# BoChenUIUC/FastVideoCodec

Measured on AMD Instinct MI355X. Metric: 1080p frames/sec encode+decode at λ=1024; bpp/PSNR parity vs CPU ref, higher is better.
Workload: dtype f32 (convs: fp32 operands split into fp16 hi/lo, f32 accumulate); 1 GPU; DVC P-frame encode+decode with rANS, 1920x1080 (padded 1920x1088) GOP-12, lambda=1024 slot; gops_per_gpu=16, frames_counted=P-frames only (I-frame pass-through), parallelism=gop-shard x1

## Files before the change

### fastvideocodec_amd/csrc/fvc_conv_x3.hip

```cpp
#include "fvc_common.h"
#include "fvc_dx.h"
#include <math.h>
#include <stdlib.h>

namespace {

#ifndef FVC_STORE_AUX
#define FVC_STORE_AUX 0
#endif

typedef _Float16 h8 __attribute__((ext_vector_type(8)));

constexpr int kMaxTapsX = 49;

constexpr float kLoScale = 2048.f;
#ifndef FVC_X3_KO
#define FVC_X3_KO 0
#endif
constexpr int kKO = FVC_X3_KO;
#ifndef FVC_X3_SCHED
#define FVC_X3_SCHED 0
#endif
constexpr int kSched = FVC_X3_SCHED;
#ifndef FVC_X3_ACC1
// ... 688 lines not shown
        for (int ky = 0; ky < ks; ++ky) {
          if (((py + pad - ky) % stride + stride) % stride) continue;
          for (int kx = 0; kx < ks; ++kx) {
            if (((px + pad - kx) % stride + stride) % stride) continue;
            const int t = c.ntaps[cl]++;
            c.tky[cl][t] = ky; c.tkx[cl][t] = kx;
            c.tdy[cl][t] = x3_floordiv(py + pad - ky, stride);
            c.tdx[cl][t] = x3_floordiv(px + pad - kx, stride);
          }
        }
      }
  }
  c.dymin = c.dxmin = 1 << 20;
  c.dymax = c.dxmax = -(1 << 20);
  for (int cl = 0; cl < c.nclass; ++cl)
    for (int t = 0; t < c.ntaps[cl]; ++t) {
      c.dymin = c.tdy[cl][t] < c.dymin ? c.tdy[cl][t] : c.dymin;
      c.dymax = c.tdy[cl][t] > c.dymax ? c.tdy[cl][t] : c.dymax;
      c.dxmin = c.tdx[cl][t] < c.dxmin ? c.tdx[cl][t] : c.dxmin;
      c.dxmax = c.tdx[cl][t] > c.dxmax ? c.tdx[cl][t] : c.dxmax;
    }
  c.dx = 0;
  c.wl = 0;
  if (transposed && stride == 2 && c.nclass == 4 && env_int("FVC_DX", 1) &&
      (c.cinp == 64 || c.cinp == 96 || c.cinp == 128) && (c.ntp == 2 || c.ntp == 4)) {
    int maxt = 0;
    for (int cl = 0; cl < 4; ++cl) maxt = c.ntaps[cl] > maxt ? c.ntaps[cl] : maxt;
    const int sw = fvc_dx::strip_width(c.cinp);
    const int R = sw == 16 ? 8 : (c.ntp == 4 ? 2 : 4);
    const int ir = R + (c.dymax - c.dymin), ic = sw + (c.dxmax - c.dxmin);
    if (maxt <= fvc_dx::kMaxTaps && fvc_dx::lds_bytes(c.cinp, fvc_dx::plane_pix(ir, ic)) <= 160 * 1024) {
      c.dx = 1;
      c.cc = c.cinp;
      c.nchunks = 1;
      c.nw = 8;
      c.wm = 2;
      c.wn = 2;
      c.wnmax = 2;
      c.th = R;
      long long off = 0;
      for (int cl = 0; cl < 4; ++cl) {
        c.nks[cl] = fvc_cdiv(c.ntaps[cl] * (c.cc / 8), 2);
        c.wcls[cl] = off;
        off += (long long)c.nks[cl] * c.ntp * kFrag;
      }
      c.wtotal = off;
      return true;
    }
  }
  c.cc = (c.cinp % 32 == 0) ? 32 : ((c.cinp % 16 == 0) ? 16 : 8);
  const int want_cc = env_int("FVC_X3_CC", 0);
  if ((want_cc == 8 || want_cc == 16 || want_cc == 32) && c.cinp % want_cc == 0) c.cc = want_cc;
  c.nw = 8;
  c.wm = env_int("FVC_X3_WM", (!transposed && stride == 2) ? 1 : 2) == 1 ? 1 : 2;
  c.wl = env_int("FVC_X3_WL", 0) ? 1 : 0;
  c.wnmax = (c.wm == 1 && !transposed && stride == 2 && c.ntp % 4 == 0) ? 4 : (c.ntp >= 2 ? 2 : 1);
  for (;;) {
    c.th = c.nw * c.wm;
    const int ir = (c.th - 1) * c.sin + 1 + (c.dymax - c.dymin);
    const int ic = 31 * c.sin + 1 + (c.dxmax - c.dxmin);
    size_t lds = 1024 + 2 * x3_tile_bytes(ir, ic, c.cc);
    if (c.wl) {
      int nkmax = 0;
      for (int cl = 0; cl < c.nclass; ++cl) {
        const int nk = fvc_cdiv(c.ntaps[cl] * (c.cc / 8), 2);
        nkmax = nk > nkmax ? nk : nkmax;
      }
      lds += 2 * (size_t)nkmax * c.wnmax * kFrag * 16;
    }
    if (lds <= 160 * 1024) break;
    if (c.cc > 8 && c.cinp % (c.cc / 2) == 0) c.cc /= 2;
    else if (c.wm > 1) c.wm /= 2;
    else return false;
  }
  c.nchunks = c.cinp == 4 ? 1 : c.cinp / c.cc;
  c.wn = 1;
  long long off = 0;
  for (int cl = 0; cl < c.nclass; ++cl) {
    c.nks[cl] = fvc_cdiv(c.ntaps[cl] * (c.cc / 8), 2);
    c.wcls[cl] = off;
    off += (long long)c.nchunks * c.nks[cl] * c.ntp * kFrag;
  }
  c.wtotal = off;
  return true;
}

static int x3_num_cus() {
  static int n = 0;
  if (!n) {
    int dev = 0;
    if (hipGetDevice(&dev) != hipSuccess ||
        hipDeviceGetAttribute(&n, hipDeviceAttributeMultiprocessorCount, dev) != hipSuccess || n <= 0)
      n = 256;
  }
  return n;
}

static int x3_kw(const float* w, size_t n) {
  float mx = 0.f;
  for (size_t i = 0; i < n; ++i) mx = fabsf(w[i]) > mx ? fabsf(w[i]) : mx;
  if (!(mx > 0.f) || !isfinite(mx)) return 0;
  int e;
  frexpf(mx, &e);
  int kw = 14 - e;
  return kw < -100 ? -100 : (kw > 100 ? 100 : kw);
}

template <int CC, int WM, int WN, int WG, int IOP, int POST, int NWV, int WL>
static int x3_launch(const X3Args& a, dim3 grid, size_t lds, hipStream_t s) {
  if (lds > 64 * 1024)
    (void)hipFuncSetAttribute((const void*)conv_x3_kernel<CC, WM, WN, WG, IOP, POST, NWV, WL>,
                              hipFuncAttributeMaxDynamicSharedMemorySize, (int)lds);
  hipLaunchKernelGGL((conv_x3_kernel<CC, WM, WN, WG, IOP, POST, NWV, WL>), grid, dim3(NWV * 64), lds, s, a);
  FVC_CHECK_LAUNCH();
  return 0;
}

template <int CC, int WM, int WN, int WG, int WL, int NWV = 8>
static int x3_launch_iop(int iop, int post, const X3Args& a, dim3 grid, size_t lds, hipStream_t s) {
  if (post == kPostPool) {
    if constexpr (WG == 1 && WL == 0 && WM == 2 && WN <= 2)
      return iop == FVC_IN_NONE ? x3_launch<CC, WM, WN, WG, FVC_IN_NONE, kPostPool, NWV, WL>(a, grid, lds, s) : FVC_EINVAL;
    return FVC_EINVAL;
  }
  if (post == kPostTap) {
    if constexpr (WG == 1 && WL == 0 && ((WM == 2 && WN <= 2) || (WM == 1 && WN == 4)))
      return iop == FVC_IN_NONE ? x3_launch<CC, WM, WN, WG, FVC_IN_NONE, kPostTap, NWV, WL>(a, grid, lds, s) : FVC_EINVAL;
    return FVC_EINVAL;
  }
  if (post == FVC_POST_EXP)
    return iop == FVC_IN_NONE ? x3_launch<CC, WM, WN, WG, FVC_IN_NONE, FVC_POST_EXP, NWV, WL>(a, grid, lds, s) : FVC_EINVAL;
  switch (iop) {
    case FVC_IN_NONE: return x3_launch<CC, WM, WN, WG, FVC_IN_NONE, FVC_POST_NONE, NWV, WL>(a, grid, lds, s);
    case FVC_IN_RELU: return x3_launch<CC, WM, WN, WG, FVC_IN_RELU, FVC_POST_NONE, NWV, WL>(a, grid, lds, s);
    case FVC_IN_ABS: return x3_launch<CC, WM, WN, WG, FVC_IN_ABS, FVC_POST_NONE, NWV, WL>(a, grid, lds, s);
    case FVC_IN_ROUND: return x3_launch<CC, WM, WN, WG, FVC_IN_ROUND, FVC_POST_NONE, NWV, WL>(a, grid, lds, s);
  }
  return FVC_EINVAL;
}

template <int CC, int WL>
static int x3_launch_cc(int nwv, int wm, int wn, int wg, int iop, int post, const X3Args& a, dim3 grid,
                        size_t lds, hipStream_t s) {
  if (nwv != 8) return FVC_EINVAL;
  if (wg == 2) return (wm == 4 && wn == 1 && !WL) ? x3_launch_iop<CC, 4, 1, 2, 0>(iop, post, a, grid, lds, s) : FVC_EINVAL;
  if (wm == 2 && wn == 2) return x3_launch_iop<CC, 2, 2, 1, WL>(iop, post, a, grid, lds, s);
  if (wm == 2 && wn == 1) return x3_launch_iop<CC, 2, 1, 1, WL>(iop, post, a, grid, lds, s);
  if (wm == 1 && wn == 2) return x3_launch_iop<CC, 1, 2, 1, WL>(iop, post, a, grid, lds, s);
  if (wm == 1 && wn == 1) return x3_launch_iop<CC, 1, 1, 1, WL>(iop, post, a, grid, lds, s);
  if (wm == 1 && wn == 4) return x3_launch_iop<CC, 1, 4, 1, WL>(iop, post, a, grid, lds, s);
  return FVC_EINVAL;
}

static int run_dx(const X3Cfg& c, const float* x, const void* wpack, float osc, const float* bias, const float* res,
                  float* y, int batch, int h, int w, int cout, int in_op, int act, int post_op, int cu_reserve,
                  int* ovf, int* sched, int sched_len, hipStream_t s, const void* tw, float tosc, int pcp,
                  unsigned y_bytes, unsigned x_bytes) {
  const bool tap = tw != nullptr;
  if (tap && res) return FVC_EINVAL;
  const int R = c.th;
  const int sw = fvc_dx::strip_width(c.cinp);
  const int S = R / (32 / sw);
  const int wm = tap ? 1 : 2, wn = tap ? c.ntp : 2;
  fvc_dx::DxArgs d;
  d.x = x;
  d.w = (const uint4*)wpack;
  d.bias = bias;
  d.res = res;
  d.y = y;
  d.post_exp = post_op == FVC_POST_EXP ? 1 : 0;
  d.B = batch;
  d.H = h;
  d.W = w;
  d.cout = cout;
  d.coutp = c.coutp;
  d.ntp = c.ntp;
  d.R = R;
  d.sw = sw;
  d.ir = R + (c.dymax - c.dymin);
  d.ic = sw + (c.dxmax - c.dxmin);
  d.ps = fvc_dx::plane_pix(d.ir, d.ic);
  d.dymin = c.dymin;
  d.dxmin = c.dxmin;
  d.inv_ic = 1.0f / (float)d.ic;
  d.tiles_x = fvc_cdiv(w, sw);
  d.tiles_y = fvc_cdiv(h, R);
  const long long nitems = (long long)batch * d.tiles_x * d.tiles_y;
  if (nitems >= (1LL << 30)) return FVC_EINVAL;
  d.nitems = (int)nitems;
  d.osc = osc;
  d.osc_c = osc * (1.0f / 2048.f);
  d.act_slope = act == FVC_ACT_RELU ? 0.f : (act == FVC_ACT_LRELU ? 0.1f : 1.f);
  for (int cl = 0; cl < 4; ++cl) {
    d.nks[cl] = c.nks[cl];
    d.oy0[cl] = c.oy0[cl];
    d.ox0[cl] = c.ox0[cl];
    d.wcls[cl] = c.wcls[cl];
    for (int t = 0; t <= fvc_dx::kMaxTaps; ++t)
      d.toff[cl][t] = t < c.ntaps[cl] ? (c.tdy[cl][t] - c.dymin) * d.ic + (c.tdx[cl][t] - c.dxmin) : 0;
  }
  struct WT {
    int cl, m0, n0, cost;
  };
  WT wt[64];
  int n = 0;
  for (int cl = 0; cl < 4; ++cl)
    for (int n0 = 0; n0 < c.ntp; n0 += wn)
      for (int m0 = 0; m0 < S; m0 += wm) {
        if (n >= 64) return FVC_EINVAL;
        wt[n++] = {cl, m0, n0, c.ntaps[cl]};
      }
  auto enc = [](const WT& t) { return t.cl | (t.m0 << 4) | (t.n0 << 8); };
  auto by_cost = [](WT* v, int k) {
    for (int i = 1; i < k; ++i)
      for (int j = i; j > 0 && v[j].cost > v[j - 1].cost; --j) {
        const WT t = v[j];
        v[j] = v[j - 1];
        v[j - 1] = t;
      }
  };
  int up[fvc_dx::kWaves][fvc_dx::kMaxWT], upc[fvc_dx::kWaves] = {0};
  int pp[fvc_dx::kWaves][fvc_dx::kMaxWT], ppc[fvc_dx::kWaves] = {0};
  int up_max = 0, pp_max = 1 << 30;
  {
    WT v[64];
    for (int i = 0; i < n; ++i) v[i] = wt[i];
    by_cost(v, n);
    int sl[4] = {0, 0, 0, 0}, wl[fvc_dx::kWaves] = {0};
    for (int i = 0; i < n; ++i) {
      int sm = 0;
      for (int q = 1; q < 4; ++q) sm = sl[q] < sl[sm] ? q : sm;
      int wv = wl[sm + 4] < wl[sm] ? sm + 4 : sm;
      if (upc[wv] == fvc_dx::kMaxWT) wv = wv == sm ? sm + 4 : sm;
      if (upc[wv] == fvc_dx::kMaxWT) return FVC_EINVAL;
      up[wv][upc[wv]++] = enc(v[i]);
      sl[sm] += v[i].cost;
      wl[wv] += v[i].cost;
    }
    for (int q = 0; q < 4; ++q) up_max = sl[q] > up_max ? sl[q] : up_max;
  }
  if ((S / wm) % 2 == 0) {
    WT jobs[32];
    int nj = 0;
    for (int i = 0; i + 1 < n; i += 2) jobs[nj++] = wt[i];
    int jidx[32];
    for (int i = 0; i < nj; ++i) jidx[i] = i;
    for (int i = 1; i < nj; ++i)
      for (int j = i; j > 0 && jobs[jidx[j]].cost > jobs[jidx[j - 1]].cost; --j) {
        const int t = jidx[j];
        jidx[j] = jidx[j - 1];
        jidx[j - 1] = t;
      }
    int sl[4] = {0, 0, 0, 0};
    bool ok = true;
    for (int i = 0; i < nj && ok; ++i) {
      const int j = jidx[i];
      int sm = 0;
      for (int q = 1; q < 4; ++q) sm = sl[q] < sl[sm] ? q : sm;
      if (ppc[sm] == fvc_dx::kMaxWT) {
        ok = false;
        break;
      }
      pp[sm][ppc[sm]++] = enc(wt[2 * j]);
      pp[sm + 4][ppc[sm + 4]++] = enc(wt[2 * j + 1]);
      sl[sm] += 2 * jobs[j].cost;
    }
    if (ok) {
      pp_max = 0;
      for (int q = 0; q < 4; ++q) pp_max = sl[q] > pp_max ? sl[q] : pp_max;
    }
  }
  const int pair_env = env_int("FVC_DX_PAIR", -1);
  const bool paired = pp_max < (1 << 30) && (pair_env == 1 || (pair_env != 0 && pp_max * 100 <= up_max * 115));
  for (int wv = 0; wv < fvc_dx::kWaves; ++wv)
    for (int j = 0; j < fvc_dx::kMaxWT; ++j)
      d.wt[wv][j] = paired ? (j < ppc[wv] ? pp[wv][j] : -1) : (j < upc[wv] ? up[wv][j] : -1);
  d.y_bytes = y_bytes;
  d.x_bytes = x_bytes;
  d.ovf = ovf;
  d.tw = (const uint4*)tw;
  d.tosc = tosc;
  d.tosc_c = tosc * (1.0f / 2048.f);
  d.pcp = pcp;
  const int reserve = env_int("FVC_X3_RESERVE", -1) >= 0 ? env_int("FVC_X3_RESERVE", 0) : cu_reserve;
  const int ncu = x3_num_cus() - (reserve < x3_num_cus() / 2 ? reserve : x3_num_cus() / 2);
  const int grid = ncu < d.nitems ? ncu : d.nitems;
  d.sched = (sched && sched_len >= 2 && env_int("FVC_X3_DYN", 1)) ? sched : nullptr;
  const size_t lds = fvc_dx::lds_bytes(c.cinp, d.ps);
  return fvc_dx::launch(d, c.cinp, wm, wn, in_op, tap, grid, lds, s);
}

static int run_x3(const float* x, const void* wpack, float osc, const float* bias, const float* res,
                  float* y, int batch, int h, int w, int cin, int cout, int ks, int stride, int transposed,
                  int in_op, int act, int post_op, int cu_reserve, int* ovf, int* sched, int sched_len,
                  hipStream_t s, const void* tw = nullptr, float tosc = 0.f, int pcp = 0, float* pool = nullptr) {
  X3Cfg c;
  if (!x3_cfg(cin, cout, ks, stride, transposed, c)) return FVC_EINVAL;
  if (!x || !wpack || !bias || !y || batch <= 0 || h <= 0 || w <= 0) return FVC_EINVAL;
  if (tw) {
    if (post_op != FVC_POST_NONE || in_op != FVC_IN_NONE || c.wl || c.ntp == 3 || c.ntp > 4 || pcp <= 0 ||
        pcp > 32 || (pcp & 3) || (c.dx && c.ntp != 4))
      return FVC_EINVAL;
    if (!c.dx) {
      if (c.ntp == 4) c.wm = 1;
      c.th = c.nw * c.wm;
    }
    post_op = kPostTap;
  }
  if (pool) {
    if (tw || transposed || stride != 1 || post_op != FVC_POST_NONE || in_op != FVC_IN_NONE || c.wl || c.wm != 2 ||
        c.ntp > 2)
      return FVC_EINVAL;
    post_op = kPostPool;
  }
  const int ych = tw ? pcp : c.coutp;
  X3Args a;
  a.x = x; a.w = (const uint4*)wpack; a.bias = bias; a.res = res; a.y = y;
  a.tw = (const uint4*)tw; a.pcp = pcp;
  a.tosc = tosc; a.tosc_c = tosc * (1.0f / 2048.f);
  a.B = batch; a.H = h; a.W = w; a.cinp = c.cinp;
  a.coutp = c.coutp; a.cout = cout;
  if (!transposed) {
    if (stride == 2 && ((h & 1) || (w & 1))) return FVC_EINVAL;
    a.Ho = h / stride; a.Wo = w / stride;
    a.Hq = a.Ho; a.Wq = a.Wo;
  } else {
    a.Ho = h * stride; a.Wo = w * stride;
    a.Hq = h; a.Wq = w;
  }
  const unsigned long long ybytes = (unsigned long long)batch * a.Ho * a.Wo * ych * 4ull;
  const unsigned long long rbytes = (unsigned long long)batch * a.Ho * a.Wo * a.coutp * 4ull;
  const long long split_env = env_int("FVC_X3_SPLIT_BYTES", 0);
  const unsigned long long split_at = split_env > 0 ? (unsigned long long)split_env : (1ull << 32) - 4096;
  if (ybytes >= split_at || (res && rbytes >= split_at)) {
    if (batch == 1) return FVC_EINVAL;
    const int b1 = batch / 2;
    const size_t xs = (size_t)h * w * c.cinp, ys = (size_t)a.Ho * a.Wo * ych, rs = (size_t)a.Ho * a.Wo * c.coutp;
    const int post_in = (tw || pool) ? FVC_POST_NONE : post_op;
    const size_t pls = (size_t)(a.Ho / 2) * (a.Wo / 2) * c.coutp;
    int rc = run_x3(x, wpack, osc, bias, res, y, b1, h, w, cin, cout, ks, stride, transposed, in_op, act,
                    post_in, cu_reserve, ovf, sched, sched_len, s, tw, tosc, pcp, pool);
    if (rc) return rc;
    return run_x3(x + b1 * xs, wpack, osc, bias, res ? res + b1 * rs : nullptr, y + b1 * ys, batch - b1, h, w, cin, cout, ks,
                  stride, transposed, in_op, act, post_in, cu_reserve, ovf, sched, sched_len, s, tw, tosc, pcp,
                  pool ? pool + b1 * pls : nullptr);
  }
  a.y_bytes = (unsigned)ybytes;
  a.res_bytes = (unsigned)rbytes;
  a.pool = pool;
  a.pool_bytes = (unsigned)((unsigned long long)batch * (a.Ho / 2) * (a.Wo / 2) * c.coutp * 4ull);
  const unsigned long long xbytes = (unsigned long long)h * w * c.cinp * 4ull;
  if (xbytes >= (1ull << 32) - 4096) return FVC_EINVAL;
  a.x_bytes = (unsigned)xbytes;
  a.ovf = ovf;
  if (c.dx)
    return run_dx(c, x, wpack, osc, bias, res, y, batch, h, w, cout, in_op, act, post_op, cu_reserve, ovf, sched,
                  sched_len, s, tw, tosc, pcp, a.y_bytes, a.x_bytes);
  a.sin = c.sin; a.sout = c.sout; a.nclass = c.nclass; a.nchunks = c.nchunks; a.ntp = c.ntp;
  a.dymin = c.dymin; a.dxmin = c.dxmin;
  const int th = c.th;
// ... 274 lines not shown
```

### fastvideocodec_amd/csrc/fvc_deconv_x3.hip

```cpp
#include "fvc_dx.h"
#include <math.h>

namespace fvc_dx {

#ifndef FVC_STORE_AUX
#define FVC_STORE_AUX 0
#endif
namespace {

typedef _Float16 h8 __attribute__((ext_vector_type(8)));
typedef float f2v __attribute__((ext_vector_type(2)));
typedef _Float16 h2v __attribute__((ext_vector_type(2)));
typedef unsigned v4u __attribute__((ext_vector_type(4)));

constexpr float kLoScale = 2048.f;
constexpr unsigned kOob = 0xFFFFFF00u;
constexpr int kRsrcFlags = 0x00020000;
constexpr int kNT = 512;
constexpr int kFrag = 128;
constexpr int kHdr = 1024;
#ifndef FVC_DX_KO
#define FVC_DX_KO 0
#endif
constexpr int kKO = FVC_DX_KO;

template <int IOP>
__device__ __forceinline__ float in_op_t(float v) {
  if (IOP == FVC_IN_RELU) return fmaxf(v, 0.f);
  if (IOP == FVC_IN_ABS) return fabsf(v);
  if (IOP == FVC_IN_ROUND) return rintf(v);
  return v;
}

__device__ __forceinline__ void split8(const float (&v)[8], h8& hi, h8& lo, float& mx) {
#pragma unroll
  for (int i = 0; i < 8; i += 2) {
    const f2v x = {v[i], v[i + 1]};
    const h2v h = __builtin_convertvector(x, h2v);
    const f2v back = __builtin_convertvector(h, f2v);
    const h2v l = __builtin_convertvector((x - back) * kLoScale, h2v);
    hi[i] = h[0];
    hi[i + 1] = h[1];
    lo[i] = l[0];
    lo[i + 1] = l[1];
  }
  mx = fmaxf(mx, fmaxf(fmaxf(fmaxf(fabsf(v[0]), fabsf(v[1])), fmaxf(fabsf(v[2]), fabsf(v[3]))),
                       fmaxf(fmaxf(fabsf(v[4]), fabsf(v[5])), fmaxf(fabsf(v[6]), fabsf(v[7])))));
}

__device__ __forceinline__ __amdgpu_buffer_rsrc_t rsrc(const void* p, unsigned bytes) {
  return __builtin_amdgcn_make_buffer_rsrc(const_cast<void*>(p), (short)0, (int)bytes, kRsrcFlags);
}

template <int CIN, int WM, int WN, int IOP, bool TAP, int SW>
__global__ __launch_bounds__(kNT) void conv_dx_kernel(const DxArgs a) {
  static_assert(SW == 32 || SW == 16, "strip shapes: 1 x 32 or 2 x 16 input pixels");
  constexpr int SR = 32 / SW;
  constexpr int C8 = CIN / 8;
  constexpr int KPT = C8 / 2;
  static_assert(C8 % 2 == 0, "a k-step's two octets must belong to one tap");

  extern __shared__ __attribute__((aligned(16))) _Float16 smh[];
  float* const sbias = reinterpret_cast<float*>(smh);
  _Float16* const sdump = smh + 256;
  int* const squeue = reinterpret_cast<int*>(smh) + 144;
  _Float16* const tile0 = smh + kHdr / 2;

  const int tid = threadIdx.x;
  const int lane = tid & 63;
  const int wave = __builtin_amdgcn_readfirstlane(tid >> 6);
  const int li = lane & 31;
  const int lh = lane >> 5;
  const int sdr = SW == 32 ? 0 : (li >> 4);
  const int sdc = SW == 32 ? li : (li < 16 ? li : ((li - 17) & 15));
  const int psh = a.ps * 8;
  const int tile_h = 2 * C8 * psh;
  const int Ho = 2 * a.H, Wo = 2 * a.W;
  const int tile_items = a.ir * a.ic * C8;
  const int nstage = (tile_items + kNT - 1) / kNT;
  float mx = 0.f;

  int* const ctr = a.sched ? a.sched + 1 : nullptr;
  auto take = [&](int k) -> int {
    if (ctr) return atomicAdd(ctr, 1);
    return (int)blockIdx.x + k * (int)gridDim.x;
  };
  auto finish = [&]() {
    if (ctr && tid == 0) {
      __threadfence();
      if (atomicAdd(a.sched, 1) == (int)gridDim.x - 1) {
        atomicExch(a.sched + 1, 0);
        atomicExch(a.sched, 0);
      }
    }
  };
  auto decode = [&](int it, int& b, int& ty0, int& tx0) {
    const int per = a.tiles_x * a.tiles_y;
    b = it / per;
    const int r = it - b * per;
    const int ty = r / a.tiles_x;
    ty0 = ty * a.R;
    tx0 = (r - ty * a.tiles_x) * SW;
  };

  struct Stage {
    float4 v0, v1;
    int dst;
    bool ok;
  };
  auto fetch = [&](int e, const __amdgpu_buffer_rsrc_t& rx, int iy0, int ix0, Stage& st) {
    if constexpr ((kKO & 2) != 0) return;
    st.ok = e < tile_items;
    e = st.ok ? e : tile_items - 1;
    const int p = e / C8;
    const int o = e - p * C8;
    const int r = (int)(((float)p + 0.5f) * a.inv_ic);
    const int c = p - r * a.ic;
    const int iy = iy0 + r, ix = ix0 + c;
    const bool inb = (unsigned)iy < (unsigned)a.H && (unsigned)ix < (unsigned)a.W;
    const unsigned off = inb ? ((unsigned)(iy * a.W + ix) * (unsigned)CIN + (unsigned)(o * 8)) * 4u : kOob;
    st.v0 = __builtin_bit_cast(float4, __builtin_amdgcn_raw_buffer_load_b128(rx, off, 0, 0));
    st.v1 = __builtin_bit_cast(float4, __builtin_amdgcn_raw_buffer_load_b128(rx, off + 16u, 0, 0));
    st.dst = o * psh + p * 8;
  };
  auto store = [&](_Float16* t, const Stage& st) {
    if constexpr ((kKO & 2) != 0) return;
    float v[8] = {st.v0.x, st.v0.y, st.v0.z, st.v0.w, st.v1.x, st.v1.y, st.v1.z, st.v1.w};
#pragma unroll
    for (int i = 0; i < 8; ++i) v[i] = in_op_t<IOP>(v[i]);
    h8 hi, lo;
    split8(v, hi, lo, mx);
    _Float16* const ph = st.ok ? t + st.dst : sdump;
    _Float16* const pl = st.ok ? t + st.dst + C8 * psh : sdump + 8;
    *reinterpret_cast<h8*>(ph) = hi;
    *reinterpret_cast<h8*>(pl) = lo;
  };
  auto image_rsrc = [&](int b) {
    return rsrc(a.x + (size_t)b * a.H * a.W * CIN, a.x_bytes);
  };

  if (tid == 0) {
    squeue[0] = take(0);
    squeue[1] = take(1);
  }
  if (tid < a.coutp) sbias[tid] = tid < a.cout ? a.bias[tid] : 0.f;
  __syncthreads();
  const int first = squeue[0];
  if (first >= a.nitems) {
    finish();
    return;
  }
  int b, ty0, tx0;
  decode(first, b, ty0, tx0);
  {
    const __amdgpu_buffer_rsrc_t rx = image_rsrc(b);
    for (int e = tid; e < tile_items; e += kNT) {
      Stage st;
      fetch(e, rx, ty0 + a.dymin, tx0 + a.dxmin, st);
      store(tile0, st);
    }
  }
  __syncthreads();

  const __amdgpu_buffer_rsrc_t ry = rsrc(a.y, a.y_bytes);
  const __amdgpu_buffer_rsrc_t rr = rsrc(a.res, a.res ? a.y_bytes : 0u);
  int buf = 0;
  for (int k = 0;; ++k) {
    const int it = squeue[k & 3];
    if (it >= a.nitems) break;
    int taken = 0;
    if (tid == 0) taken = take(k + 2);
    decode(it, b, ty0, tx0);
    const int s_it = squeue[(k + 1) & 3];
    const bool stage_next = s_it < a.nitems;
    int sb = 0, sty0 = 0, stx0 = 0;
    if (stage_next) decode(s_it, sb, sty0, stx0);
    const __amdgpu_buffer_rsrc_t rxs = image_rsrc(sb);
    const int siy0 = sty0 + a.dymin, six0 = stx0 + a.dxmin;
    const _Float16* const cur = tile0 + buf * tile_h;
    _Float16* const nxt = tile0 + (buf ^ 1) * tile_h;
    int staged = 0;

    for (int j = 0; j < kMaxWT; ++j) {
      const int ent = a.wt[wave][j];
      if (ent < 0) break;
      const int cls = ent & 15, m0 = (ent >> 4) & 15, n0 = (ent >> 8) & 15;
      const int nq = a.nks[cls];
      const int tap_tab = a.toff[cls][lane <= kMaxTaps ? lane : kMaxTaps];
      const uint4* const wcl = a.w + a.wcls[cls] + lane;
      int pix[WM];
#pragma unroll
      for (int m = 0; m < WM; ++m) pix[m] = (((m0 + m) * SR + sdr) * a.ic + sdc) * 8;

      f32x16 acc[WM][WN], cor[WM][WN];
#pragma unroll
      for (int m = 0; m < WM; ++m)
#pragma unroll
        for (int n = 0; n < WN; ++n)
#pragma unroll
          for (int r = 0; r < 16; ++r) acc[m][n][r] = cor[m][n][r] = 0.f;

      struct Ops {
        h8 ah[WM], al[WM];
        uint4 bh[WN], bl[WN];
      };
      auto load = [&](int q, Ops& op) {
        const int t = q / KPT;
        const int toffh = __builtin_amdgcn_readlane(tap_tab, t) * 8 + (2 * (q - t * KPT) + lh) * psh;
#pragma unroll
        for (int m = 0; m < WM; ++m) {
          if constexpr ((kKO & 4) != 0) {
            op.ah[m] = h8{} + (_Float16)(q + m + toffh);
            op.al[m] = h8{} + (_Float16)(q);
            continue;
          }
          op.ah[m] = *reinterpret_cast<const h8*>(cur + toffh + pix[m]);
          op.al[m] = *reinterpret_cast<const h8*>(cur + toffh + pix[m] + C8 * psh);
        }
        const uint4* const wk = wcl + ((size_t)q * a.ntp + n0) * kFrag;
#pragma unroll
        for (int n = 0; n < WN; ++n) {
          if constexpr ((kKO & 1) != 0) {
            op.bh[n] = uint4{(unsigned)(q + n), 1u, 2u, 3u};
            op.bl[n] = uint4{(unsigned)q, 5u, 6u, 7u};
            continue;
          }
          op.bh[n] = wk[n * kFrag];
          op.bl[n] = wk[n * kFrag + 64];
        }
      };
      auto mfmas = [&](const Ops& op) {
        if constexpr ((kKO & 8) != 0) {
#pragma unroll
          for (int m = 0; m < WM; ++m)
#pragma unroll
            for (int n = 0; n < WN; ++n)
              acc[m][n][0] += (float)op.ah[m][0] + (float)op.al[m][1] + __builtin_bit_cast(float, op.bh[n].x) +
                              __builtin_bit_cast(float, op.bl[n].y);
          return;
        }
#pragma unroll
        for (int m = 0; m < WM; ++m)
#pragma unroll
          for (int n = 0; n < WN; ++n) {
            const h8 wh = __builtin_bit_cast(h8, op.bh[n]);
            const h8 wl = __builtin_bit_cast(h8, op.bl[n]);
            acc[m][n] = __builtin_amdgcn_mfma_f32_32x32x16_f16(wh, op.ah[m], acc[m][n], 0, 0, 0);
            cor[m][n] = __builtin_amdgcn_mfma_f32_32x32x16_f16(wl, op.ah[m], cor[m][n], 0, 0, 0);
            cor[m][n] = __builtin_amdgcn_mfma_f32_32x32x16_f16(wh, op.al[m], cor[m][n], 0, 0, 0);
          }
      };
      auto pin = []() { __builtin_amdgcn_sched_barrier(0); };
      Ops S0, S1;
      load(0, S0);
      const int npair = nq >> 1;
      const int nst = stage_next ? min(nstage - staged, npair) : 0;
      const int spread = nst ? max(1, npair / nst) : 1;
      int q = 0;
      for (int s = 0; s < nst; ++s) {
        load(q + 1, S1);
        Stage st;
        fetch(tid + (staged + s) * kNT, rxs, siy0, six0, st);
        pin();
        mfmas(S0);
        pin();
        load(q + 2 < nq ? q + 2 : nq - 1, S0);
        pin();
        mfmas(S1);
        pin();
        store(nxt, st);
        q += 2;
        for (int r = 1; r < spread && q < nq; ++r, q += 2) {
          load(q + 1, S1);
          pin();
          mfmas(S0);
          pin();
          load(q + 2 < nq ? q + 2 : nq - 1, S0);
          pin();
          mfmas(S1);
          pin();
        }
      }
      staged += nst;
      for (; q < nq; q += 2) {
        load(q + 1, S1);
        pin();
        mfmas(S0);
        pin();
        load(q + 2 < nq ? q + 2 : nq - 1, S0);
        pin();
        mfmas(S1);
        pin();
      }

      const int oyc = a.oy0[cls], oxc = a.ox0[cls];
      const int col = tx0 + sdc;
      if constexpr (TAP) {
#pragma unroll
        for (int m = 0; m < WM; ++m) {
          const int row = ty0 + (m0 + m) * SR + sdr;
          const bool ok = row < a.H && col < a.W;
          const unsigned pixo = ((unsigned)b * Ho + 2 * row + oyc) * (unsigned)Wo + 2 * col + oxc;
          f32x16 pa, pc;
#pragma unroll
          for (int r = 0; r < 16; ++r) pa[r] = pc[r] = 0.f;
#pragma unroll
          for (int n = 0; n < WN; ++n) {
            float yv[16];
#pragma unroll
            for (int g = 0; g < 4; ++g) {
              const float4 bj = *reinterpret_cast<const float4*>(sbias + (n0 + n) * 32 + 8 * g + 4 * lh);
              const float bb[4] = {bj.x, bj.y, bj.z, bj.w};
#pragma unroll
              for (int i = 0; i < 4; ++i) {
                const int r = 4 * g + i;
                const float tv = fmaf(cor[m][n][r], a.osc_c, fmaf(acc[m][n][r], a.osc, bb[i]));
                yv[r] = fmaxf(tv, tv * a.act_slope);
              }
            }
#pragma unroll
            for (int gp = 0; gp < 2; ++gp) {
              float v8[8];
#pragma unroll
              for (int t = 0; t < 8; ++t) v8[t] = yv[8 * gp + t];
              h8 yh, yl;
              split8(v8, yh, yl, mx);
              const uint4* const tw = a.tw + (size_t)(((n0 + n) * 2 + gp) * 2) * 64 + lane;
              const h8 wh = __builtin_bit_cast(h8, tw[0]);
              const h8 wl = __builtin_bit_cast(h8, tw[64]);
              pa = __builtin_amdgcn_mfma_f32_32x32x16_f16(wh, yh, pa, 0, 0, 0);
              pc = __builtin_amdgcn_mfma_f32_32x32x16_f16(wl, yh, pc, 0, 0, 0);
              pc = __builtin_amdgcn_mfma_f32_32x32x16_f16(wh, yl, pc, 0, 0, 0);
            }
          }
          const unsigned po = pixo * (unsigned)a.pcp * 4u + (unsigned)(4 * lh) * 4u;
#pragma unroll
          for (int g = 0; g < 4; ++g) {
            const int p0 = 8 * g + 4 * lh;
            float o[4];
#pragma unroll
            for (int i = 0; i < 4; ++i) o[i] = fmaf(pc[4 * g + i], a.tosc_c, pa[4 * g + i] * a.tosc);
            const unsigned so = (ok && p0 < a.pcp && !(kKO & 16)) ? po + 32u * g : kOob;
            __builtin_amdgcn_raw_buffer_store_b128(__builtin_bit_cast(v4u, make_float4(o[0], o[1], o[2], o[3])), ry,
                                                   so, 0, 0);
          }
        }
      } else {
#pragma unroll
        for (int m = 0; m < WM; ++m) {
          const int row = ty0 + (m0 + m) * SR + sdr;
          const bool ok = row < a.H && col < a.W;
          const unsigned pixo = ((unsigned)b * Ho + 2 * row + oyc) * (unsigned)Wo + 2 * col + oxc;
#pragma unroll
          for (int n = 0; n < WN; ++n) {
            const unsigned vo = pixo * (unsigned)a.coutp * 4u + (unsigned)((n0 + n) * 32 + 4 * lh) * 4u;
            float4 rq[4];
            if (a.res) {
#pragma unroll
              for (int g = 0; g < 4; ++g)
                rq[g] = __builtin_bit_cast(float4, __builtin_amdgcn_raw_buffer_load_b128(rr, vo + 32u * g, 0, 0));
            }
#pragma unroll
            for (int g = 0; g < 4; ++g) {
              const int j0 = (n0 + n) * 32 + 8 * g + 4 * lh;
              const float4 bj = *reinterpret_cast<const float4*>(sbias + j0);
              const float bb[4] = {bj.x, bj.y, bj.z, bj.w};
              float v[4];
#pragma unroll
              for (int i = 0; i < 4; ++i) {
                const int r = 4 * g + i;
                const float tv = fmaf(cor[m][n][r], a.osc_c, fmaf(acc[m][n][r], a.osc, bb[i]));
                v[i] = fmaxf(tv, tv * a.act_slope);
              }
              if (a.res) {
                v[0] += rq[g].x;
                v[1] += rq[g].y;
                v[2] += rq[g].z;
                v[3] += rq[g].w;
              }
              if (a.post_exp) {
#pragma unroll
                for (int i = 0; i < 4; ++i) v[i] = j0 + i < a.cout ? expf(v[i]) : 0.f;
              }
              const unsigned so = (ok && j0 < a.coutp && !(kKO & 16)) ? vo + 32u * g : kOob;
              __builtin_amdgcn_raw_buffer_store_b128(__builtin_bit_cast(v4u, make_float4(v[0], v[1], v[2], v[3])),
                                                     ry, so, 0, FVC_STORE_AUX);
            }
          }
        }
      }
    }
    if (stage_next) {
      for (; staged < nstage; ++staged) {
        Stage st;
        fetch(tid + staged * kNT, rxs, siy0, six0, st);
        store(nxt, st);
      }
    }
    if (tid == 0) squeue[(k + 2) & 3] = taken;
    __syncthreads();
    buf ^= 1;
  }
  if (!(mx < 65000.f) && a.ovf) atomicOr(a.ovf, 1);
  finish();
}

template <int CIN, int WM, int WN, int IOP, bool TAP>
int launch_t(const DxArgs& a, int grid, size_t lds, hipStream_t s) {
  constexpr int SW = CIN == 128 ? 16 : 32;
  if (a.sw != SW) return FVC_EINVAL;
  const hipError_t e = hipFuncSetAttribute((const void*)conv_dx_kernel<CIN, WM, WN, IOP, TAP, SW>,
                                           hipFuncAttributeMaxDynamicSharedMemorySize, (int)lds);
  if (e != hipSuccess) return -(int)e;
  hipLaunchKernelGGL((conv_dx_kernel<CIN, WM, WN, IOP, TAP, SW>), dim3(grid), dim3(kNT), lds, s, a);
  FVC_CHECK_LAUNCH();
  return 0;
}

template <int CIN>
int launch_cin(const DxArgs& a, int wm, int wn, int iop, bool tap, int grid, size_t lds, hipStream_t s) {
  if (tap) {
    if constexpr (CIN == 128)
      if (wm == 1 && wn == 4 && iop == FVC_IN_NONE) return launch_t<CIN, 1, 4, FVC_IN_NONE, true>(a, grid, lds, s);
    return FVC_EINVAL;
  }
  if (wm != 2 || wn != 2) return FVC_EINVAL;
  switch (iop) {
    case FVC_IN_NONE: return launch_t<CIN, 2, 2, FVC_IN_NONE, false>(a, grid, lds, s);
    case FVC_IN_RELU: return launch_t<CIN, 2, 2, FVC_IN_RELU, false>(a, grid, lds, s);
    case FVC_IN_ABS: return launch_t<CIN, 2, 2, FVC_IN_ABS, false>(a, grid, lds, s);
    case FVC_IN_ROUND: return launch_t<CIN, 2, 2, FVC_IN_ROUND, false>(a, grid, lds, s);
  }
  return FVC_EINVAL;
}

}

size_t lds_bytes(int cinp, int ps) { return (size_t)kHdr + 2 * (size_t)cinp * 4 * (size_t)ps; }

int plane_pix(int ir, int ic) { return (ir * ic) | 1; }

int launch(const DxArgs& a, int cinp, int wm, int wn, int iop, bool tap, int grid, size_t lds, hipStream_t s) {
  if (grid <= 0 || lds > 160 * 1024) return FVC_EINVAL;
  switch (cinp) {
    case 64: return launch_cin<64>(a, wm, wn, iop, tap, grid, lds, s);
    case 96: return launch_cin<96>(a, wm, wn, iop, tap, grid, lds, s);
    case 128: return launch_cin<128>(a, wm, wn, iop, tap, grid, lds, s);
  }
  return FVC_EINVAL;
}

}
```

Before: 81.58 P-frames/s.

## Retile fused-tap deconv to 2 pixel strips x 1 channel block looped over channels

For the deconv kernel with a fused 1x1 tail conv, the default tile changes from 1 strip x 4 output-channel blocks to 2 strips x 1 channel block. The kernel walks the 4 channel blocks sequentially and folds each into per-strip tail accumulators. Each weight fragment is now reused across two pixel strips, and the live accumulator set is smaller, which should ease register pressure. The cost is that the main K loop, including its staging interleave, runs four times per work tile, and the input tile loads are repeated for each channel block.

```diff
diff --git a/fastvideocodec_amd/csrc/fvc_conv_x3.hip b/fastvideocodec_amd/csrc/fvc_conv_x3.hip
--- a/fastvideocodec_amd/csrc/fvc_conv_x3.hip
+++ b/fastvideocodec_amd/csrc/fvc_conv_x3.hip
@@ -864,6 +864,7 @@
   return FVC_EINVAL;
 }
 
+constexpr int kDxTileDefault = 1;
 static int run_dx(const X3Cfg& c, const float* x, const void* wpack, float osc, const float* bias, const float* res,
                   float* y, int batch, int h, int w, int cout, int in_op, int act, int post_op, int cu_reserve,
                   int* ovf, int* sched, int sched_len, hipStream_t s, const void* tw, float tosc, int pcp,
@@ -873,7 +874,9 @@
   const int R = c.th;
   const int sw = fvc_dx::strip_width(c.cinp);
   const int S = R / (32 / sw);
-  const int wm = tap ? 1 : 2, wn = tap ? c.ntp : 2;
+  const bool tap2 = tap && S % 2 == 0 && env_int("FVC_DX_TILE", kDxTileDefault) != 0;
+  const int wm = tap ? (tap2 ? 2 : 1) : 2, wn = tap ? (tap2 ? 1 : c.ntp) : 2;
+  const int wn_span = tap ? c.ntp : wn;
   fvc_dx::DxArgs d;
   d.x = x;
   d.w = (const uint4*)wpack;
@@ -917,7 +920,7 @@
   WT wt[64];
   int n = 0;
   for (int cl = 0; cl < 4; ++cl)
-    for (int n0 = 0; n0 < c.ntp; n0 += wn)
+    for (int n0 = 0; n0 < c.ntp; n0 += wn_span)
       for (int m0 = 0; m0 < S; m0 += wm) {
         if (n >= 64) return FVC_EINVAL;
         wt[n++] = {cl, m0, n0, c.ntaps[cl]};
diff --git a/fastvideocodec_amd/csrc/fvc_deconv_x3.hip b/fastvideocodec_amd/csrc/fvc_deconv_x3.hip
--- a/fastvideocodec_amd/csrc/fvc_deconv_x3.hip
+++ b/fastvideocodec_amd/csrc/fvc_deconv_x3.hip
@@ -59,6 +59,7 @@
   constexpr int C8 = CIN / 8;
   constexpr int KPT = C8 / 2;
   static_assert(C8 % 2 == 0, "a k-step's two octets must belong to one tap");
+  constexpr int NP = TAP ? 4 / WN : 1;
 
   extern __shared__ __attribute__((aligned(16))) _Float16 smh[];
   float* const sbias = reinterpret_cast<float*>(smh);
@@ -184,208 +185,221 @@
     for (int j = 0; j < kMaxWT; ++j) {
       const int ent = a.wt[wave][j];
       if (ent < 0) break;
-      const int cls = ent & 15, m0 = (ent >> 4) & 15, n0 = (ent >> 8) & 15;
+      const int cls = ent & 15, m0 = (ent >> 4) & 15, nb = (ent >> 8) & 15;
       const int nq = a.nks[cls];
+      const int oyc = a.oy0[cls], oxc = a.ox0[cls];
+      const int col = tx0 + sdc;
       const int tap_tab = a.toff[cls][lane <= kMaxTaps ? lane : kMaxTaps];
       const uint4* const wcl = a.w + a.wcls[cls] + lane;
       int pix[WM];
 #pragma unroll
       for (int m = 0; m < WM; ++m) pix[m] = (((m0 + m) * SR + sdr) * a.ic + sdc) * 8;
 
-      f32x16 acc[WM][WN], cor[WM][WN];
-#pragma unroll
-      for (int m = 0; m < WM; ++m)
-#pragma unroll
-        for (int n = 0; n < WN; ++n)
-#pragma unroll
-          for (int r = 0; r < 16; ++r) acc[m][n][r] = cor[m][n][r] = 0.f;
-
-      struct Ops {
-        h8 ah[WM], al[WM];
-        uint4 bh[WN], bl[WN];
-      };
-      auto load = [&](int q, Ops& op) {
-        const int t = q / KPT;
-        const int toffh = __builtin_amdgcn_readlane(tap_tab, t) * 8 + (2 * (q - t * KPT) + lh) * psh;
-#pragma unroll
-        for (int m = 0; m < WM; ++m) {
-          if constexpr ((kKO & 4) != 0) {
-            op.ah[m] = h8{} + (_Float16)(q + m + toffh);
-            op.al[m] = h8{} + (_Float16)(q);
-            continue;
-          }
-          op.ah[m] = *reinterpret_cast<const h8*>(cur + toffh + pix[m]);
-          op.al[m] = *reinterpret_cast<const h8*>(cur + toffh + pix[m] + C8 * psh);
+      f32x16 pa[TAP ? WM : 1], pc[TAP ? WM : 1];
+      if constexpr (TAP) {
+#pragma unroll
+        for (int m = 0; m < WM; ++m)
+#pragma unroll
+          for (int r = 0; r < 16; ++r) pa[m][r] = pc[m][r] = 0.f;
+      }
+#pragma unroll 1
+      for (int np = 0; np < NP; ++np) {
+        const int n0 = nb + np * WN;
+        f32x16 acc[WM][WN], cor[WM][WN];
+#pragma unroll
+        for (int m = 0; m < WM; ++m)
+#pragma unroll
+          for (int n = 0; n < WN; ++n)
+#pragma unroll
+            for (int r = 0; r < 16; ++r) acc[m][n][r] = cor[m][n][r] = 0.f;
+
+        struct Ops {
+          h8 ah[WM], al[WM];
+          uint4 bh[WN], bl[WN];
+        };
+        auto load = [&](int q, Ops& op) {
+          const int t = q / KPT;
+          const int toffh = __builtin_amdgcn_readlane(tap_tab, t) * 8 + (2 * (q - t * KPT) + lh) * psh;
+#pragma unroll
+          for (int m = 0; m < WM; ++m) {
+            if constexpr ((kKO & 4) != 0) {
+              op.ah[m] = h8{} + (_Float16)(q + m + toffh);
+              op.al[m] = h8{} + (_Float16)(q);
+              continue;
+            }
+            op.ah[m] = *reinterpret_cast<const h8*>(cur + toffh + pix[m]);
+            op.al[m] = *reinterpret_cast<const h8*>(cur + toffh + pix[m] + C8 * psh);
+          }
+          const uint4* const wk = wcl + ((size_t)q * a.ntp + n0) * kFrag;
+#pragma unroll
+          for (int n = 0; n < WN; ++n) {
+            if constexpr ((kKO & 1) != 0) {
+              op.bh[n] = uint4{(unsigned)(q + n), 1u, 2u, 3u};
+              op.bl[n] = uint4{(unsigned)q, 5u, 6u, 7u};
+              continue;
+            }
+            op.bh[n] = wk[n * kFrag];
+            op.bl[n] = wk[n * kFrag + 64];
+          }
+        };
+        auto mfmas = [&](const Ops& op) {
+          if constexpr ((kKO & 8) != 0) {
+#pragma unroll
+            for (int m = 0; m < WM; ++m)
+#pragma unroll
+              for (int n = 0; n < WN; ++n)
+                acc[m][n][0] += (float)op.ah[m][0] + (float)op.al[m][1] + __builtin_bit_cast(float, op.bh[n].x) +
+                                __builtin_bit_cast(float, op.bl[n].y);
+            return;
+          }
+#pragma unroll
+          for (int m = 0; m < WM; ++m)
+#pragma unroll
+            for (int n = 0; n < WN; ++n) {
+              const h8 wh = __builtin_bit_cast(h8, op.bh[n]);
+              const h8 wl = __builtin_bit_cast(h8, op.bl[n]);
+              acc[m][n] = __builtin_amdgcn_mfma_f32_32x32x16_f16(wh, op.ah[m], acc[m][n], 0, 0, 0);
+              cor[m][n] = __builtin_amdgcn_mfma_f32_32x32x16_f16(wl, op.ah[m], cor[m][n], 0, 0, 0);
+              cor[m][n] = __builtin_amdgcn_mfma_f32_32x32x16_f16(wh, op.al[m], cor[m][n], 0, 0, 0);
+            }
+        };
+        auto pin = []() { __builtin_amdgcn_sched_barrier(0); };
+        Ops S0, S1;
+        load(0, S0);
+        const int npair = nq >> 1;
+        const int nst = stage_next ? min(nstage - staged, npair) : 0;
+        const int spread = nst ? max(1, npair / nst) : 1;
+        int q = 0;
+        for (int s = 0; s < nst; ++s) {
+          load(q + 1, S1);
+          Stage st;
+          fetch(tid + (staged + s) * kNT, rxs, siy0, six0, st);
+          pin();
+          mfmas(S0);
+          pin();
+          load(q + 2 < nq ? q + 2 : nq - 1, S0);
+          pin();
+          mfmas(S1);
+          pin();
+          store(nxt, st);
+          q += 2;
+          for (int r = 1; r < spread && q < nq; ++r, q += 2) {
+            load(q + 1, S1);
+            pin();
+            mfmas(S0);
+            pin();
+            load(q + 2 < nq ? q + 2 : nq - 1, S0);
+            pin();
+            mfmas(S1);
+            pin();
+          }
         }
-        const uint4* const wk = wcl + ((size_t)q * a.ntp + n0) * kFrag;
-#pragma unroll
-        for (int n = 0; n < WN; ++n) {
-          if constexpr ((kKO & 1) != 0) {
-            op.bh[n] = uint4{(unsigned)(q + n), 1u, 2u, 3u};
-            op.bl[n] = uint4{(unsigned)q, 5u, 6u, 7u};
-            continue;
-          }
-          op.bh[n] = wk[n * kFrag];
-          op.bl[n] = wk[n * kFrag + 64];
+        staged += nst;
+        for (; q < nq; q += 2) {
+          load(q + 1, S1);
+          pin();
+          mfmas(S0);
+          pin();
+          load(q + 2 < nq ? q + 2 : nq - 1, S0);
+          pin();
+          mfmas(S1);
+          pin();
         }
-      };
-      auto mfmas = [&](const Ops& op) {
-        if constexpr ((kKO & 8) != 0) {
-#pragma unroll
-          for (int m = 0; m < WM; ++m)
-#pragma unroll
-            for (int n = 0; n < WN; ++n)
-              acc[m][n][0] += (float)op.ah[m][0] + (float)op.al[m][1] + __builtin_bit_cast(float, op.bh[n].x) +
-                              __builtin_bit_cast(float, op.bl[n].y);
-          return;
-        }
-#pragma unroll
-        for (int m = 0; m < WM; ++m)
-#pragma unroll
-          for (int n = 0; n < WN; ++n) {
-            const h8 wh = __builtin_bit_cast(h8, op.bh[n]);
-            const h8 wl = __builtin_bit_cast(h8, op.bl[n]);
-            acc[m][n] = __builtin_amdgcn_mfma_f32_32x32x16_f16(wh, op.ah[m], acc[m][n], 0, 0, 0);
-            cor[m][n] = __builtin_amdgcn_mfma_f32_32x32x16_f16(wl, op.ah[m], cor[m][n], 0, 0, 0);
-            cor[m][n] = __builtin_amdgcn_mfma_f32_32x32x16_f16(wh, op.al[m], cor[m][n], 0, 0, 0);
-          }
-      };
-      auto pin = []() { __builtin_amdgcn_sched_barrier(0); };
-      Ops S0, S1;
-      load(0, S0);
-      const int npair = nq >> 1;
-      const int nst = stage_next ? min(nstage - staged, npair) : 0;
-      const int spread = nst ? max(1, npair / nst) : 1;
-      int q = 0;
-      for (int s = 0; s < nst; ++s) {
-        load(q + 1, S1);
-        Stage st;
-        fetch(tid + (staged + s) * kNT, rxs, siy0, six0, st);
-        pin();
-        mfmas(S0);
-        pin();
-        load(q + 2 < nq ? q + 2 : nq - 1, S0);
-        pin();
-        mfmas(S1);
-        pin();
-        store(nxt, st);
-        q += 2;
-        for (int r = 1; r < spread && q < nq; ++r, q += 2) {
-          load(q + 1, S1);
-          pin();
-          mfmas(S0);
-          pin();
-          load(q + 2 < nq ? q + 2 : nq - 1, S0);
-          pin();
-          mfmas(S1);
-          pin();
+
+        if constexpr (TAP) {
+#pragma unroll
+          for (int m = 0; m < WM; ++m) {
+#pragma unroll
+            for (int n = 0; n < WN; ++n) {
+              float yv[16];
+#pragma unroll
+              for (int g = 0; g < 4; ++g) {
+                const float4 bj = *reinterpret_cast<const float4*>(sbias + (n0 + n) * 32 + 8 * g + 4 * lh);
+                const float bb[4] = {bj.x, bj.y, bj.z, bj.w};
+#pragma unroll
+                for (int i = 0; i < 4; ++i) {
+                  const int r = 4 * g + i;
+                  const float tv = fmaf(cor[m][n][r], a.osc_c, fmaf(acc[m][n][r], a.osc, bb[i]));
+                  yv[r] = fmaxf(tv, tv * a.act_slope);
+                }
+              }
+#pragma unroll
+              for (int gp = 0; gp < 2; ++gp) {
+                float v8[8];
+#pragma unroll
+                for (int t = 0; t < 8; ++t) v8[t] = yv[8 * gp + t];
+                h8 yh, yl;
+                split8(v8, yh, yl, mx);
+                const uint4* const tw = a.tw + (size_t)(((n0 + n) * 2 + gp) * 2) * 64 + lane;
+                const h8 wh = __builtin_bit_cast(h8, tw[0]);
+                const h8 wl = __builtin_bit_cast(h8, tw[64]);
+                pa[m] = __builtin_amdgcn_mfma_f32_32x32x16_f16(wh, yh, pa[m], 0, 0, 0);
+                pc[m] = __builtin_amdgcn_mfma_f32_32x32x16_f16(wl, yh, pc[m], 0, 0, 0);
+                pc[m] = __builtin_amdgcn_mfma_f32_32x32x16_f16(wh, yl, pc[m], 0, 0, 0);
+              }
+            }
+          }
+        } else {
+#pragma unroll
+          for (int m = 0; m < WM; ++m) {
+            const int row = ty0 + (m0 + m) * SR + sdr;
+            const bool ok = row < a.H && col < a.W;
+            const unsigned pixo = ((unsigned)b * Ho + 2 * row + oyc) * (unsigned)Wo + 2 * col + oxc;
+#pragma unroll
+            for (int n = 0; n < WN; ++n) {
+              const unsigned vo = pixo * (unsigned)a.coutp * 4u + (unsigned)((n0 + n) * 32 + 4 * lh) * 4u;
+              float4 rq[4];
+              if (a.res) {
+#pragma unroll
+                for (int g = 0; g < 4; ++g)
+                  rq[g] = __builtin_bit_cast(float4, __builtin_amdgcn_raw_buffer_load_b128(rr, vo + 32u * g, 0, 0));
+              }
+#pragma unroll
+              for (int g = 0; g < 4; ++g) {
+                const int j0 = (n0 + n) * 32 + 8 * g + 4 * lh;
+                const float4 bj = *reinterpret_cast<const float4*>(sbias + j0);
+                const float bb[4] = {bj.x, bj.y, bj.z, bj.w};
+                float v[4];
+#pragma unroll
+                for (int i = 0; i < 4; ++i) {
+                  const int r = 4 * g + i;
+                  const float tv = fmaf(cor[m][n][r], a.osc_c, fmaf(acc[m][n][r], a.osc, bb[i]));
+                  v[i] = fmaxf(tv, tv * a.act_slope);
+                }
+                if (a.res) {
+                  v[0] += rq[g].x;
+                  v[1] += rq[g].y;
+                  v[2] += rq[g].z;
+                  v[3] += rq[g].w;
+                }
+                if (a.post_exp) {
+#pragma unroll
+                  for (int i = 0; i < 4; ++i) v[i] = j0 + i < a.cout ? expf(v[i]) : 0.f;
+                }
+                const unsigned so = (ok && j0 < a.coutp && !(kKO & 16)) ? vo + 32u * g : kOob;
+                __builtin_amdgcn_raw_buffer_store_b128(__builtin_bit_cast(v4u, make_float4(v[0], v[1], v[2], v[3])),
+                                                       ry, so, 0, FVC_STORE_AUX);
+              }
+            }
+          }
         }
       }
-      staged += nst;
-      for (; q < nq; q += 2) {
-        load(q + 1, S1);
-        pin();
-        mfmas(S0);
-        pin();
-        load(q + 2 < nq ? q + 2 : nq - 1, S0);
-        pin();
-        mfmas(S1);
-        pin();
-      }
-
-      const int oyc = a.oy0[cls], oxc = a.ox0[cls];
-      const int col = tx0 + sdc;
       if constexpr (TAP) {
 #pragma unroll
         for (int m = 0; m < WM; ++m) {
           const int row = ty0 + (m0 + m) * SR + sdr;
           const bool ok = row < a.H && col < a.W;
           const unsigned pixo = ((unsigned)b * Ho + 2 * row + oyc) * (unsigned)Wo + 2 * col + oxc;
-          f32x16 pa, pc;
-#pragma unroll
-          for (int r = 0; r < 16; ++r) pa[r] = pc[r] = 0.f;
-#pragma unroll
-          for (int n = 0; n < WN; ++n) {
-            float yv[16];
-#pragma unroll
-            for (int g = 0; g < 4; ++g) {
-              const float4 bj = *reinterpret_cast<const float4*>(sbias + (n0 + n) * 32 + 8 * g + 4 * lh);
-              const float bb[4] = {bj.x, bj.y, bj.z, bj.w};
-#pragma unroll
-              for (int i = 0; i < 4; ++i) {
-                const int r = 4 * g + i;
-                const float tv = fmaf(cor[m][n][r], a.osc_c, fmaf(acc[m][n][r], a.osc, bb[i]));
-                yv[r] = fmaxf(tv, tv * a.act_slope);
-              }
-            }
-#pragma unroll
-            for (int gp = 0; gp < 2; ++gp) {
-              float v8[8];
-#pragma unroll
-              for (int t = 0; t < 8; ++t) v8[t] = yv[8 * gp + t];
-              h8 yh, yl;
-              split8(v8, yh, yl, mx);
-              const uint4* const tw = a.tw + (size_t)(((n0 + n) * 2 + gp) * 2) * 64 + lane;
-              const h8 wh = __builtin_bit_cast(h8, tw[0]);
-              const h8 wl = __builtin_bit_cast(h8, tw[64]);
-              pa = __builtin_amdgcn_mfma_f32_32x32x16_f16(wh, yh, pa, 0, 0, 0);
-              pc = __builtin_amdgcn_mfma_f32_32x32x16_f16(wl, yh, pc, 0, 0, 0);
-              pc = __builtin_amdgcn_mfma_f32_32x32x16_f16(wh, yl, pc, 0, 0, 0);
-            }
-          }
           const unsigned po = pixo * (unsigned)a.pcp * 4u + (unsigned)(4 * lh) * 4u;
 #pragma unroll
           for (int g = 0; g < 4; ++g) {
             const int p0 = 8 * g + 4 * lh;
             float o[4];
 #pragma unroll
-            for (int i = 0; i < 4; ++i) o[i] = fmaf(pc[4 * g + i], a.tosc_c, pa[4 * g + i] * a.tosc);
+            for (int i = 0; i < 4; ++i) o[i] = fmaf(pc[m][4 * g + i], a.tosc_c, pa[m][4 * g + i] * a.tosc);
             const unsigned so = (ok && p0 < a.pcp && !(kKO & 16)) ? po + 32u * g : kOob;
             __builtin_amdgcn_raw_buffer_store_b128(__builtin_bit_cast(v4u, make_float4(o[0], o[1], o[2], o[3])), ry,
                                                    so, 0, 0);
-          }
-        }
-      } else {
-#pragma unroll
-        for (int m = 0; m < WM; ++m) {
-          const int row = ty0 + (m0 + m) * SR + sdr;
-          const bool ok = row < a.H && col < a.W;
-          const unsigned pixo = ((unsigned)b * Ho + 2 * row + oyc) * (unsigned)Wo + 2 * col + oxc;
-#pragma unroll
-          for (int n = 0; n < WN; ++n) {
-            const unsigned vo = pixo * (unsigned)a.coutp * 4u + (unsigned)((n0 + n) * 32 + 4 * lh) * 4u;
-            float4 rq[4];
-            if (a.res) {
-#pragma unroll
-              for (int g = 0; g < 4; ++g)
-                rq[g] = __builtin_bit_cast(float4, __builtin_amdgcn_raw_buffer_load_b128(rr, vo + 32u * g, 0, 0));
-            }
-#pragma unroll
-            for (int g = 0; g < 4; ++g) {
-              const int j0 = (n0 + n) * 32 + 8 * g + 4 * lh;
-              const float4 bj = *reinterpret_cast<const float4*>(sbias + j0);
-              const float bb[4] = {bj.x, bj.y, bj.z, bj.w};
-              float v[4];
-#pragma unroll
-              for (int i = 0; i < 4; ++i) {
-                const int r = 4 * g + i;
-                const float tv = fmaf(cor[m][n][r], a.osc_c, fmaf(acc[m][n][r], a.osc, bb[i]));
-                v[i] = fmaxf(tv, tv * a.act_slope);
-              }
-              if (a.res) {
-                v[0] += rq[g].x;
-                v[1] += rq[g].y;
-                v[2] += rq[g].z;
-                v[3] += rq[g].w;
-              }
-              if (a.post_exp) {
-#pragma unroll
-                for (int i = 0; i < 4; ++i) v[i] = j0 + i < a.cout ? expf(v[i]) : 0.f;
-              }
-              const unsigned so = (ok && j0 < a.coutp && !(kKO & 16)) ? vo + 32u * g : kOob;
-              __builtin_amdgcn_raw_buffer_store_b128(__builtin_bit_cast(v4u, make_float4(v[0], v[1], v[2], v[3])),
-                                                     ry, so, 0, FVC_STORE_AUX);
-            }
           }
         }
       }
@@ -420,8 +434,11 @@
 template <int CIN>
 int launch_cin(const DxArgs& a, int wm, int wn, int iop, bool tap, int grid, size_t lds, hipStream_t s) {
   if (tap) {
-    if constexpr (CIN == 128)
-      if (wm == 1 && wn == 4 && iop == FVC_IN_NONE) return launch_t<CIN, 1, 4, FVC_IN_NONE, true>(a, grid, lds, s);
+    if constexpr (CIN == 128) {
+      if (a.ntp != 4 || iop != FVC_IN_NONE) return FVC_EINVAL;
+      if (wm == 1 && wn == 4) return launch_t<CIN, 1, 4, FVC_IN_NONE, true>(a, grid, lds, s);
+      if (wm == 2 && wn == 1) return launch_t<CIN, 2, 1, FVC_IN_NONE, true>(a, grid, lds, s);
+    }
     return FVC_EINVAL;
   }
   if (wm != 2 || wn != 2) return FVC_EINVAL;
```

Result: no change. 82.12 P-frames/s, median of 6 (+0.7%).
